# emilk/field_interpolation

Measured on NVIDIA B200. Metric: 3D SDF solve: lattice cells x CG iterations per second, higher is better.
Workload: dtype f32

## Files before the change

### field_interpolation_b200/csrc/solver.cu

```cuda
#include "solver.hpp"

#include <algorithm>
#include <cmath>
#include <cstdlib>

namespace fi {

namespace {

constexpr int kThreads = 256;

int vec_grid(int64_t n)
{
	const int64_t want = (n + kThreads - 1) / kThreads;
	return static_cast<int>(std::max<int64_t>(1, std::min<int64_t>(want, static_cast<int64_t>(sm_count()) * 8)));
}

template <typename T>
struct Pack;
template <>
struct Pack<float>
{
	using type = float4;
	static constexpr int V = 4;
// ... 17 lines not shown
	}
}

template <typename T, typename F>
__device__ __forceinline__ void for_each_pack_blocked(int64_t n, int64_t* first, int64_t* last, F&& f)
{
	constexpr int V      = Pack<T>::V;
	const int64_t npacks = n / V;
	const int64_t chunk  = (npacks + gridDim.x - 1) / gridDim.x;
	const int64_t k0 = static_cast<int64_t>(blockIdx.x) * chunk, k1 = min(k0 + chunk, npacks);
	for (int64_t k = k0 + threadIdx.x; k < k1; k += blockDim.x) { f(k, true); }
	*first = k0 * V;
	*last  = k1 * V;
	if (blockIdx.x == gridDim.x - 1) {
		for (int64_t i = npacks * V + threadIdx.x; i < n; i += blockDim.x) { f(i, false); }
		*last = n;
	}
}

template <typename T>
__global__ void __launch_bounds__(kThreads) pcg_init_kernel(int64_t n, const T* __restrict__ b, const T* __restrict__ q,
                                                            const T* __restrict__ minv, T* __restrict__ r, T* __restrict__ p,
                                                            PcgState* st, double tol, long long max_iters, double* partial,
                                                            unsigned* ticket, int dist)
{
	__shared__ double red[32];
	double            acc[3] = {0, 0, 0};
	const int64_t     stride = static_cast<int64_t>(gridDim.x) * blockDim.x;
	for (int64_t i = static_cast<int64_t>(blockIdx.x) * blockDim.x + threadIdx.x; i < n; i += stride) {
		const T bi = b[i], ri = q ? bi - q[i] : bi, zi = minv[i] * ri;
		r[i] = ri;
		p[i] = zi;
		acc[0] += static_cast<double>(ri) * static_cast<double>(zi);
		acc[1] += static_cast<double>(ri) * static_cast<double>(ri);
		acc[2] += static_cast<double>(bi) * static_cast<double>(bi);
	}
	acc[0] = block_sum(acc[0], red);
	acc[1] = block_sum(acc[1], red);
	acc[2] = block_sum(acc[2], red);
	grid_sum<3>(acc, partial, ticket, red, [&](const double(&tot)[3]) {
		if (dist) {
			st->part[0] = tot[0];
			st->part[1] = tot[1];
			st->part[2] = tot[2];
			return;
		}
		st->rho[0]    = tot[0];
		st->rho[1]    = 0;
		st->pq        = 0;
		st->rr        = tot[1];
		st->rr0       = tot[1];
		st->bb        = tot[2];
		st->tol2bb    = tol * tol * tot[2];
		st->iters     = 0;
// ... 138 lines not shown
	});
	acc[0] = block_sum(acc[0], red);
	acc[1] = block_sum(acc[1], red);
	grid_sum<2>(acc, partial, ticket, red, [&](const double(&tot)[2]) {
		if (XM == kXSkip) { st->alpha_prev = alpha_d; }
		if (dist) {
			st->part[0] = tot[0];
			st->part[1] = tot[1];
			return;
		}
		st->rho[par ^ 1] = tot[0];
		st->rr           = tot[1];
		st->iters += 1;
		if (tot[1] <= st->tol2bb || st->iters >= st->max_iters || !(tot[0] > 0.0)) { st->done = 1; }
	});
}

template <typename T>
struct DirRing
{
	const T* p[kMaxXRing];
};

template <typename T, int M, bool PACKED>
__device__ __forceinline__ void ring_update_elements(int64_t k, T* __restrict__ x, T* __restrict__ r, const DirRing<T>& d, const T* __restrict__ q,
                                                     const T* __restrict__ minv, T alpha, const T (&a)[kMaxXRing], double (&acc)[2])
{
	using P         = typename Pack<T>::type;
	constexpr int V = PACKED ? Pack<T>::V : 1;
	constexpr int MD = M > 0 ? M : 1;
	T ra[V], qa[V], ma[V], xa[V], da[MD][V];
	if (PACKED) {
		*reinterpret_cast<P*>(ra) = reinterpret_cast<const P*>(r)[k];
		*reinterpret_cast<P*>(qa) = reinterpret_cast<const P*>(q)[k];
		*reinterpret_cast<P*>(ma) = reinterpret_cast<const P*>(minv)[k];
		if (M > 0) {
			*reinterpret_cast<P*>(xa) = reinterpret_cast<const P*>(x)[k];
#pragma unroll
			for (int j = 0; j < M; ++j) { *reinterpret_cast<P*>(da[j]) = reinterpret_cast<const P*>(d.p[j])[k]; }
		}
	} else {
		ra[0] = r[k];
		qa[0] = q[k];
		ma[0] = minv[k];
		if (M > 0) {
			xa[0] = x[k];
#pragma unroll
			for (int j = 0; j < M; ++j) { da[j][0] = d.p[j][k]; }
		}
	}
#pragma unroll
	for (int e = 0; e < V; ++e) {
		if (M > 0) {
			T s = a[0] * da[0][e];
#pragma unroll
			for (int j = 1; j < M; ++j) { s += a[j] * da[j][e]; }
			xa[e] += s;
		}
		ra[e] -= alpha * qa[e];
		const double rd = static_cast<double>(ra[e]);
		acc[0] += rd * static_cast<double>(ma[e] * ra[e]);
		acc[1] += rd * rd;
	}
	if (PACKED) {
		if (M > 0) { reinterpret_cast<P*>(x)[k] = *reinterpret_cast<const P*>(xa); }
		reinterpret_cast<P*>(r)[k] = *reinterpret_cast<const P*>(ra);
	} else {
		if (M > 0) { x[k] = xa[0]; }
		r[k] = ra[0];
	}
}

template <typename T, int M>
__global__ void __launch_bounds__(kThreads) pcg_update_ring_kernel(int64_t n, T* __restrict__ x, T* __restrict__ r, DirRing<T> d,
                                                                   const T* __restrict__ q, const T* __restrict__ minv, PcgState* st, int par,
                                                                   double* __restrict__ alpha, int pos, double* partial, unsigned* ticket)
{
	__shared__ double red[32];
	if (st->done) { return; }
	const double pq = st->pq;
	if (!(pq > 0.0)) {
		if (blockIdx.x == 0 && threadIdx.x == 0) {
			st->breakdown = 1;
			st->done      = 1;
		}
		return;
	}
	const double alpha_d = st->rho[par] / pq;
	T            a[kMaxXRing];
#pragma unroll
	for (int j = 0; j < kMaxXRing; ++j) { a[j] = j < M - 1 ? static_cast<T>(alpha[j]) : T(0); }
	if (M > 0) { a[M > 0 ? M - 1 : 0] = static_cast<T>(alpha_d); }
	double acc[2] = {0, 0};
	for_each_pack<T>(n, [&](int64_t k, bool packed) {
		if (packed) {
			ring_update_elements<T, M, true>(k, x, r, d, q, minv, static_cast<T>(alpha_d), a, acc);
		} else {
			ring_update_elements<T, M, false>(k, x, r, d, q, minv, static_cast<T>(alpha_d), a, acc);
		}
	});
	acc[0] = block_sum(acc[0], red);
	acc[1] = block_sum(acc[1], red);
	grid_sum<2>(acc, partial, ticket, red, [&](const double(&tot)[2]) {
		if (M == 0) { alpha[pos] = alpha_d; }
		st->rho[par ^ 1] = tot[0];
		st->rr           = tot[1];
		st->iters += 1;
		if (tot[1] <= st->tol2bb || st->iters >= st->max_iters || !(tot[0] > 0.0)) { st->done = 1; }
	});
}

template <typename T, int XM>
__global__ void __launch_bounds__(kThreads) pcg_update_peer_kernel(int64_t n, T* __restrict__ x, T* __restrict__ r,
                                                                   const T* __restrict__ p, const T* __restrict__ p_prev, const T* __restrict__ q,
                                                                   const T* __restrict__ minv, PcgState* st, int par, double* partial,
                                                                   unsigned* ticket, PeerLink L, HaloPush<T> push, unsigned long long base, int fold,
                                                                   int blocked)
{
	__shared__ double red[32];
	__shared__ double s_pq, s_tot[2];
	__shared__ int    s_ok, s_pub;
// ... 185 lines not shown
		FI_REQUIRE(m == 2 || m == 4 || m == 8, FI_ERR_INVALID, "FI_B200_X_RING must be 2, 4 or 8");
	} else {
		int dev = 0, l2 = 0;
		FI_CUDA(cudaGetDevice(&dev));
		FI_CUDA(cudaDeviceGetAttribute(&l2, cudaDevAttrL2CacheSize, dev));
		const size_t l2_bytes = l2 > 0 ? static_cast<size_t>(l2) : static_cast<size_t>(126) << 20;
		if (6 * vec <= l2_bytes) { return 2; }
	}
	size_t free_b = 0, total_b = 0;
	FI_CUDA(cudaMemGetInfo(&free_b, &total_b));
	while (m > 2 && static_cast<size_t>(std::max(0, m - op.work.dirs)) * vec > free_b / 2) { m /= 2; }
	return m;
}

template <typename T>
void ensure_ring(PcgWork<T>& w, size_t n, int m, cudaStream_t s)
{
	for (; w.dirs < m; ++w.dirs) {
		w.dir[w.dirs].resize(n);
		w.dir[w.dirs].zero(s);
	}
}

template <typename T>
void launch_ring_update(PcgWork<T>& w, int m, int pos, int grid, int64_t n, T* x, const T* minv, int par, cudaStream_t s)
{
	DirRing<T> d = {};
	if (pos < m - 1) {
		auto ku = pcg_update_ring_kernel<T, 0>;
		FI_LAUNCH(ku, grid, kThreads, 0, s, n, x, w.r.data(), d, w.q.data(), minv, w.state.data(), par, w.alpha.data(), pos, w.partial.data(),
		          w.ticket.data());
		return;
	}
	for (int j = 0; j < m; ++j) { d.p[j] = w.dir[(j + 1) % m].data(); }
	auto ku = m == 8 ? pcg_update_ring_kernel<T, 8> : m == 4 ? pcg_update_ring_kernel<T, 4> : pcg_update_ring_kernel<T, 2>;
	FI_LAUNCH(ku, grid, kThreads, 0, s, n, x, w.r.data(), d, w.q.data(), minv, w.state.data(), par, w.alpha.data(), pos, w.partial.data(),
	          w.ticket.data());
}

template <typename T>
void ensure_work(Operator<T>& op, cudaStream_t s)
{
	PcgWork<T>& w = op.work;
	const size_t n = static_cast<size_t>(op.g.N);
	if (w.r.size() != n) {
		w.r.resize(n);
		w.q.resize(n);
		for (int j = 2; j < kMaxXRing; ++j) { w.dir[j].release(); }
		w.dirs = 0;
		ensure_ring(w, n, 2, s);
		w.alpha.resize(kMaxXRing - 1);
		if (op.g.sharded()) {
			w.r.zero(s);
			w.q.zero(s);
		}
		w.partial.resize(static_cast<size_t>(3) * (static_cast<size_t>(sm_count()) * 8 + 8));
		w.ticket.resize(1);
		w.state.resize(1);
		w.ticket.zero(s);
	}
// ... 72 lines not shown
PcgResult pcg_solve(Operator<T>& op, const T* b, T* x, double tol, long long max_iter, int check_every, bool want_true_residual,
                    cudaStream_t s)
{
	TraceScope trace("pcg_solve");
	ensure_work(op, s);
	PcgWork<T>&   w = op.work;
	const int64_t off = op.g.own_offset(), n = op.g.own_cells();
	DistHooks*    dist = op.dist;
	const T*      rhs = b ? b : op.atb.data();
	if (max_iter <= 0) {
		max_iter = 2 * static_cast<long long>(op.g.size[0]) * op.g.size[1] * op.g.size[2];
	}
	if (!(tol > 0)) { tol = std::is_same<T, float>::value ? 1.1920929e-07 : 2.220446049250313e-16; }
	const int ring = choose_x_ring(op);
	ensure_ring(w, static_cast<size_t>(op.g.N), ring, s);
	check_every = std::max(ring, check_every <= 0 ? 32 : check_every);
	check_every = (check_every + ring - 1) / ring * ring;

	cudaEvent_t e0, e1;
	FI_CUDA(cudaEventCreate(&e0));
	FI_CUDA(cudaEventCreate(&e1));
	FI_CUDA(cudaEventRecord(e0, s));

	const int grid = vec_grid(n);
	const PeerLink* link = dist ? dist->link() : nullptr;
	T*              r_vec = w.r.data();
	HaloPush<T>     push;
	if (link) {
		void *lo = nullptr, *hi = nullptr;
		r_vec = static_cast<T*>(dist->shared_vector(static_cast<size_t>(op.g.N) * sizeof(T), &lo, &hi, s));
		const int64_t plane = op.g.stride[2], halo = op.g.zown0;
		push.count = halo * plane;
		if (lo) { push.lo = static_cast<T*>(lo) + halo * plane + dist->peer_own_cells(link->rank - 1); }
		if (hi) { push.hi = static_cast<T*>(hi); }
	}
	const bool zero_guess = op.guess_is_zero;
	op.guess_is_zero      = false;
	if (!zero_guess) {
		if (dist) { dist->exchange_halo(x, sizeof(T), s); }
		op.apply(x, w.q.data(), nullptr, nullptr, s);
	}
	{
		auto kern = pcg_init_kernel<T>;
		FI_LAUNCH(kern, grid, kThreads, 0, s, n, rhs + off, zero_guess ? static_cast<const T*>(nullptr) : w.q.data() + off, op.minv.data() + off, r_vec + off, w.dir[0].data() + off,
		          w.state.data(), tol, max_iter, w.partial.data(), w.ticket.data(), dist ? 1 : 0);
		if (dist) {
			dist->allreduce(w.state.data()->part, 3, s);
			FI_LAUNCH(pcg_init_finish_kernel, 1, 1, 0, s, w.state.data(), tol, max_iter);
			dist->exchange_halo(r_vec, sizeof(T), s);
		}
	}
	PcgState h;
	FI_CUDA(cudaMemcpyAsync(&h, w.state.data(), sizeof(h), cudaMemcpyDeviceToHost, s));
	FI_CUDA(cudaStreamSynchronize(s));

	PcgResult res;
	res.zero_rhs         = (h.bb == 0.0);
	res.initial_residual = h.bb > 0 ? std::sqrt(h.rr0 / h.bb) : 0.0;
	if (res.zero_rhs) {
		FI_CUDA(cudaMemsetAsync(x + off, 0, n * sizeof(T), s));
	} else if (!h.done) {
		const int* d_done = &w.state.data()->done;
		double*    d_pq   = &w.state.data()->pq;
		const unsigned long long seq_base = link ? (dist->next_seq() << 40) : 0ull;
		const char* fold_env  = std::getenv("FI_B200_PEER_FOLD");
		const int   fold_mode = !link ? 0 : (fold_env && *fold_env >= '0' && *fold_env <= '3' ? *fold_env - '0' : 2);
		const bool  data_publishes = fold_mode >= 2, update_finishes = fold_mode == 1 || fold_mode == 2;
		const char* walk_env = std::getenv("FI_B200_PEER_UPDATE");
		const bool  peer_update_blocked = walk_env ? walk_env[0] == 'b' : n < (48ll << 20);
		bool deferred_x = false;
		auto enqueue_round = [&] {
			for (int it = 0; it < check_every; ++it) {
				const int par = it & 1, pos = it % ring;
				T* const   p_old = w.dir[pos].data();
				T* const   p_new = w.dir[(pos + 1) % ring].data();
				const bool fused = stencil_fused_step<T>(op.use_fast, op.g, op.tabs, r_vec, op.minv.data(), p_old, p_new, w.q.data(),
				                                         w.state.data(), par, d_pq, op.partial.data(), op.ticket.data(), d_done, s);
				deferred_x = deferred_x || fused;
				if (fused && link) {
					PeerPublish pub;
					pub.link  = *link;
					pub.which = 0;
					pub.par   = par;
					pub.base  = seq_base;
					pub.st    = w.state.data();
					const bool published = apply_data_term<T>(op.g, op.data, p_new, w.q.data(), d_pq, d_done, s, data_publishes ? &pub : nullptr);
					const bool in_update = fold_mode == 1;
					if (!published && !in_update) { FI_LAUNCH(peer_publish_kernel, 1, 32, 0, s, *link, 0, par, seq_base, w.state.data(), d_pq, 1, d_done); }
					auto ku = par == 0 ? pcg_update_peer_kernel<T, kXSkip> : pcg_update_peer_kernel<T, kXBoth>;
					FI_LAUNCH(ku, grid, kThreads, 0, s, n, x + off, r_vec + off, p_new + off, p_old + off, w.q.data() + off, op.minv.data() + off,
					          w.state.data(), par, w.partial.data(), w.ticket.data(), *link, push, seq_base, (in_update ? 1 : 0) | (update_finishes ? 2 : 0),
					          peer_update_blocked ? 1 : 0);
					if (!update_finishes) { FI_LAUNCH(pcg_update_finish_peer_kernel, 1, 32, 0, s, w.state.data(), par, *link, seq_base); }
				} else if (fused && !dist) {
					apply_data_term<T>(op.g, op.data, p_new, w.q.data(), d_pq, d_done, s);
					launch_ring_update<T>(w, ring, pos, grid, n, x, op.minv.data(), par, s);
				} else if (fused) {
					apply_data_term<T>(op.g, op.data, p_new, w.q.data(), d_pq, d_done, s);
					if (dist) { dist->allreduce(d_pq, 1, s); }
					auto ku = par == 0 ? pcg_update_kernel<T, kXSkip> : pcg_update_kernel<T, kXBoth>;
					FI_LAUNCH(ku, grid, kThreads, 0, s, n, x + off, r_vec + off, p_new + off, p_old + off, w.q.data() + off, op.minv.data() + off,
					          w.state.data(), par, w.partial.data(), w.ticket.data(), dist ? 1 : 0);
					if (dist) {
						dist->allreduce(w.state.data()->part, 2, s);
						FI_LAUNCH(pcg_update_finish_kernel, 1, 1, 0, s, w.state.data(), par);
						dist->exchange_halo(r_vec, sizeof(T), s);
					}
				} else {
					FI_REQUIRE(dist == nullptr, FI_ERR_UNSUPPORTED, "a slab-sharded solve needs the fused 3D stencil kernel");
					T* const p = w.dir[0].data();
					op.apply(p, w.q.data(), d_pq, d_done, s);
					auto ku = pcg_update_kernel<T, kXClassic>;
					FI_LAUNCH(ku, grid, kThreads, 0, s, n, x, w.r.data(), p, static_cast<const T*>(nullptr), w.q.data(), op.minv.data(), w.state.data(), par,
					          w.partial.data(), w.ticket.data(), 0);
					auto kd = pcg_direction_kernel<T>;
					FI_LAUNCH(kd, grid, kThreads, 0, s, n, w.r.data(), op.minv.data(), p, w.state.data(), par);
				}
			}
		};
// ... 194 lines not shown
	h.alpha_prev = 0;
	if (!(h.rho[0] > 0)) { h.rho[0] = 1; }
	if (!(h.rho[1] > 0)) { h.rho[1] = 1; }
	if (!(h.pq > 0)) { h.pq = 1; }
	FI_CUDA(cudaMemcpyAsync(w.state.data(), &h, sizeof(h), cudaMemcpyHostToDevice, s));
	FI_CUDA(cudaStreamSynchronize(s));
	cudaEvent_t e0, e1;
	FI_CUDA(cudaEventCreate(&e0));
	FI_CUDA(cudaEventCreate(&e1));
	auto timed = [&](auto&& body) {
		FI_CUDA(cudaEventRecord(e0, s));
		for (int i = 0; i < iterations; ++i) { body(i); }
		FI_CUDA(cudaEventRecord(e1, s));
		FI_CUDA(cudaEventSynchronize(e1));
		float ms = 0;
		FI_CUDA(cudaEventElapsedTime(&ms, e0, e1));
		return static_cast<double>(ms);
	};
	DevBuf<double> dot(1);
	const int m     = std::max(2, r.x_ring);
	T*        p0    = w.dir[0].data();
	auto      p_old = [&](int i) { return w.dir[i % m].data(); };
	auto      p_new = [&](int i) { return w.dir[(i + 1) % m].data(); };
	bool      fused = false;
	out[1] = timed([&](int i) {
		const int par = i & 1;
		fused = stencil_fused_step<T>(op.use_fast, op.g, op.tabs, w.r.data(), op.minv.data(), p_old(i), p_new(i), w.q.data(),
		                              w.state.data(), par, dot.data(), op.partial.data(), op.ticket.data(), nullptr, s);
		if (fused) {
			apply_data_term<T>(op.g, op.data, p_new(i), w.q.data(), dot.data(), nullptr, s);
		} else {
			op.apply(p0, w.q.data(), dot.data(), nullptr, s);
		}
	});
	h.pq = 1e30;
	FI_CUDA(cudaMemcpyAsync(w.state.data(), &h, sizeof(h), cudaMemcpyHostToDevice, s));
	FI_CUDA(cudaStreamSynchronize(s));
	out[2] = timed([&](int i) {
		if (!fused) {
			auto ku = pcg_update_kernel<T, kXClassic>;
			FI_LAUNCH(ku, vec_grid(n), kThreads, 0, s, n, x.data(), w.r.data(), p0, static_cast<const T*>(nullptr), w.q.data(), op.minv.data(), w.state.data(), 0,
			          w.partial.data(), w.ticket.data(), 0);
		} else {
			launch_ring_update<T>(w, m, i % m, vec_grid(n), n, x.data(), op.minv.data(), 0, s);
		}
	});
	out[3] = 0.0;
	if (!fused) {
		out[3] = timed([&](int) {
			auto kd = pcg_direction_kernel<T>;
			FI_LAUNCH(kd, vec_grid(n), kThreads, 0, s, n, w.r.data(), op.minv.data(), p0, w.state.data(), 0);
		});
	}
	out[4] = fused ? 1.0 : 0.0;
	out[7] = fused ? m : 1;
	out[5] = timed([&](int i) {
		const int par = i & 1;
		if (fused) {
			stencil_fused_step<T>(op.use_fast, op.g, op.tabs, w.r.data(), op.minv.data(), p_old(i), p_new(i), w.q.data(), w.state.data(), par,
			                      dot.data(), op.partial.data(), op.ticket.data(), nullptr, s);
		} else {
			stencil_apply<T>(op.g, op.tabs, p0, w.q.data(), dot.data(), op.partial.data(), op.ticket.data(), nullptr, op.use_fast, s);
		}
	});
	out[6] = timed([&](int i) {
		apply_data_term<T>(op.g, op.data, fused ? p_new(i) : p0, w.q.data(), dot.data(), nullptr, s);
	});
	cudaEventDestroy(e0);
	cudaEventDestroy(e1);
}

template void time_kernels<float>(Operator<float>&, int, int, double*, cudaStream_t);
template void time_kernels<double>(Operator<double>&, int, int, double*, cudaStream_t);
template std::unique_ptr<Operator<float>> build_operator<float>(const Geom&, const ModelAccum&, const PointStore&, const HostRows&, cudaStream_t);
template std::unique_ptr<Operator<double>> build_operator<double>(const Geom&, const ModelAccum&, const PointStore&, const HostRows&, cudaStream_t);
template PcgResult pcg_solve<float>(Operator<float>&, const float*, float*, double, long long, int, bool, cudaStream_t);
template PcgResult pcg_solve<double>(Operator<double>&, const double*, double*, double, long long, int, bool, cudaStream_t);
template PcgResult tile_phase<float>(Operator<float>&, int, float*, double, long long, int, cudaStream_t);
template PcgResult tile_phase<double>(Operator<double>&, int, double*, double, long long, int, cudaStream_t);
template void jacobi_sweeps<float>(Operator<float>&, float*, int, float, cudaStream_t);
template void jacobi_sweeps<double>(Operator<double>&, double*, int, double, cudaStream_t);
template void residual<float>(Operator<float>&, const float*, const float*, float*, double*, double*, cudaStream_t);
// ... 4 lines not shown
```

### field_interpolation_b200/csrc/solver.hpp

```cpp
#pragma once

#include <utility>
#include <vector>

#include "internal.hpp"
#include "peer.cuh"

namespace fi {

struct DistHooks
{
	virtual ~DistHooks() = default;
	virtual const PeerLink* link() { return nullptr; }
	virtual void* shared_vector(size_t bytes, void** lo, void** hi, cudaStream_t s)
	{
		(void)bytes; (void)lo; (void)hi; (void)s;
		return nullptr;
	}
	virtual int64_t peer_own_cells(int peer) { (void)peer; return 0; }
	virtual unsigned long long next_seq() { return 0; }
	virtual void allreduce(double* d_ptr, int count, cudaStream_t s) = 0;
	virtual void exchange_halo(void* d_vec, size_t elem_size, cudaStream_t s) = 0;
	virtual int rank() const { return 0; }
	virtual int world() const { return 1; }
// ... 50 lines not shown

struct PcgResult
{
	long long iterations = 0;
	double    rel_residual = 0, initial_residual = 0, true_residual = 0, solve_ms = 0;
	double    loop_ms = 0;
	int       x_ring = 1;
	bool      converged = false, zero_rhs = false;
	bool      stalled = false;
};

constexpr double kConvergedSlack = 1.25;

template <typename T>
PcgResult pcg_solve(Operator<T>& op, const T* b, T* x, double tol, long long max_iter, int check_every, bool want_true_residual,
                    cudaStream_t s);

template <typename T>
bool stencil_fast_3d_fused(const Geom& g, const StencilTables& t, const T* r, const T* minv, const T* p_old, T* p_new, T* q,
                           const PcgState* st, int par, double* d_dot_out, double* d_partial, unsigned* d_ticket, const int* d_done,
                           cudaStream_t s);

template <typename T>
bool stencil_tma_3d_fused(const Geom& g, const StencilTables& t, const T* r, const T* minv, const T* p_old, T* p_new, T* q,
                          const PcgState* st, int par, double* d_dot_out, double* d_partial, unsigned* d_ticket, const int* d_done,
                          cudaStream_t s);

template <typename T>
bool stencil_tma_3d_epilogue(const Geom& g, const StencilTables& t, const T* in, const T* res_in, T* res_out, const T* minv, T* e, T* d_new,
                             T a, T b, cudaStream_t s);

template <typename T>
bool stencil_tma_2d_fused(const Geom& g, const StencilTables& t, const T* r, const T* minv, const T* p_old, T* p_new, T* q, const PcgState* st, int par,
                          double* d_dot_out, double* d_partial, unsigned* d_ticket, const int* d_done, cudaStream_t s);
template <typename T>
bool stencil_tma_2d_epilogue(const Geom& g, const StencilTables& t, const T* in, const T* res_in, T* res_out, const T* minv, T* e, T* d_new, T a, T b,
                             cudaStream_t s);

template <typename T>
inline bool stencil_fused_step(int mode, const Geom& g, const StencilTables& t, const T* r, const T* minv, const T* p_old, T* p_new,
                               T* q, const PcgState* st, int par, double* d_dot_out, double* d_partial, unsigned* d_ticket,
                               const int* d_done, cudaStream_t s)
{
	if (g.tile) { return false; }
	if (mode == kStencilAuto && g.ndim == 2) { return stencil_tma_2d_fused<T>(g, t, r, minv, p_old, p_new, q, st, par, d_dot_out, d_partial, d_ticket, d_done, s); }
	if (mode == kStencilAuto && stencil_tma_3d_fused<T>(g, t, r, minv, p_old, p_new, q, st, par, d_dot_out, d_partial, d_ticket, d_done, s)) { return true; }
	if (mode != kStencilGeneric && stencil_fast_3d_fused<T>(g, t, r, minv, p_old, p_new, q, st, par, d_dot_out, d_partial, d_ticket, d_done, s)) { return true; }
	return false;
}

struct MgOptions
{
	int    nu               = 3;
	int    nu_coarse        = 0;
	int    gamma            = 1;
	int    w_levels         = 3;
	double cheb_ratio       = 12.0;
	int    coarsest_cells   = 600;
	int    power_iterations = 20;
	int    tail_cells       = 0;
};

inline MgOptions default_mg_options(const ModelAccum& m, const Geom& g, bool sharded, int user_nu, double user_ratio)
{
	MgOptions o;
	const bool high_order = m.on[3] || m.on[4];
	o.nu        = high_order ? 5 : 2;
	o.nu_coarse = high_order ? 0 : 4;
	const int64_t cells = static_cast<int64_t>(g.size[0]) * g.size[1] * g.size[2];
// ... 99 lines not shown
```

### field_interpolation_b200/csrc/stencil_tma.cu

```cuda
#include <cstdlib>
#include <type_traits>

#include "solver.hpp"
#include "tma.cuh"

namespace fi {

namespace {

using namespace tma;

template <typename T, int R, int TY_ = 8>
struct Tile
{
	static constexpr int V    = 16 / sizeof(T);
	static constexpr int NP   = (R + V - 1) / V;
	static constexpr int TXP  = 32;
	static constexpr int TY   = TY_;
	static constexpr int BXP  = TXP + 2 * NP;
	static constexpr int BY   = TY + 2 * R;
	__host__ __device__ static constexpr int ring(bool gs) { return R + 2 + (gs ? 1 : 0); }
	static constexpr int TILE_BYTES = ((BXP * BY * 16 + 127) / 128) * 128;
	static constexpr int BOX_BYTES  = BXP * BY * 16;
};

template <typename T, int R, int S, bool Fused, bool GS, int TY = 8>
constexpr size_t smem_bytes()
{
	using G = Tile<T, R, TY>;
	return 128  + static_cast<size_t>(S) * (Fused ? 3 : 1) * G::TILE_BYTES + static_cast<size_t>(G::ring(GS)) * G::TILE_BYTES +
	       S * sizeof(uint64_t) + 9 * (2 * R + 1) * sizeof(T) + 32 * sizeof(double) + 64;
}

template <typename T, int R, int S, bool Fused, int MINB, bool Epi, bool GS, int TY>
__global__ void __launch_bounds__(256, MINB)
    stencil3d_tma_kernel(const __grid_constant__ CUtensorMap map_a,
                         const __grid_constant__ CUtensorMap map_b,
                         const __grid_constant__ CUtensorMap map_c,
                         int nx, int ny, int nzl, int zo0, int zo1, int zoff, int nzg, int zchunk, TmaTables<T> tab, T gs2,
                         T* __restrict__ q, T* __restrict__ p_new,
                         const PcgState* st, int par, double* dot_out, double* partial, unsigned* ticket, const int* done, EpiArgs<T> epi)
{
	static_assert(!(Fused && Epi), "the epilogue mode takes a plain input");
	using G           = Tile<T, R, TY>;
	constexpr int V   = G::V;
	constexpr int NP  = G::NP;
	constexpr int NA  = Fused ? 3 : 1;
	constexpr int W   = 2 * R + 1;
	constexpr int RING = G::ring(GS);
	using Pack        = typename PackOf<T>::type;
	using PU          = PackU<T, V>;

	if (done && *done) { return; }

#ifdef FI_B200_EMU
	unsigned char* smem_raw = ::cuda_emu::dynamic_smem();
#else
	extern __shared__ unsigned char smem_raw[];
#endif
	unsigned char* base = smem_raw + ((128u - (smem_u32(smem_raw) & 127u)) & 127u);
	auto stage_ptr = [&](int s, int a) { return reinterpret_cast<Pack*>(base + (static_cast<size_t>(s) * NA + a) * G::TILE_BYTES); };
	unsigned char* ring_base = base + static_cast<size_t>(S) * NA * G::TILE_BYTES;
	auto ring_ptr = [&](int slot) { return reinterpret_cast<Pack*>(ring_base + static_cast<size_t>(slot) * G::TILE_BYTES); };
	uint64_t* full  = reinterpret_cast<uint64_t*>(ring_base + static_cast<size_t>(RING) * G::TILE_BYTES);
	T*        zband = reinterpret_cast<T*>(full + S);
	double*   red   = reinterpret_cast<double*>((reinterpret_cast<uintptr_t>(zband + 9 * W) + 7) & ~uintptr_t(7));

	const int tid = threadIdx.x, tx = tid & 31, ty = tid >> 5;
	const int x0t = blockIdx.x * (G::TXP * V);
	const int y0t = blockIdx.y * G::TY;
// ... 26 lines not shown
	}
	{
		const int cls = row_class(min(y, ny - 1), ny);
#pragma unroll
		for (int t = 0; t < W; ++t) { cy[t] = tab.band[1][cls][t + 4 - R]; }
	}
	T lx0[V], ly0 = T(0);
	if (GS) {
#pragma unroll
		for (int j = 0; j < V; ++j) {
			const int xi = min(x0 + j, nx - 1);
			lx0[j]       = static_cast<T>((xi > 0 ? 1 : 0) + (xi < nx - 1 ? 1 : 0));
		}
		const int yi = min(y, ny - 1);
		ly0          = static_cast<T>((yi > 0 ? 1 : 0) + (yi < ny - 1 ? 1 : 0));
	}

	const int lp0    = zb - R;
	const int n_iter = ze + R - lp0;
	auto issue = [&](int i) {
		const int s = i % S;
		mbar_expect_tx(&full[s], NA * G::BOX_BYTES);
		tma_load_3d(stage_ptr(s, 0), &map_a, &full[s], x0t - NP * V, y0t - R, lp0 + i);
		if (Fused) {
			tma_load_3d(stage_ptr(s, 1), &map_b, &full[s], x0t - NP * V, y0t - R, lp0 + i);
			tma_load_3d(stage_ptr(s, 2), &map_c, &full[s], x0t - NP * V, y0t - R, lp0 + i);
		}
	};
	__syncthreads();
	if (tid == 0) {
		for (int i = 0; i < S && i < n_iter; ++i) { issue(i); }
	}

	const bool has_yh = ty < 2 * R;
	const int  yh_row = ty < R ? ty : G::TY + ty;
	const bool has_xh = tid < 2 * NP * G::TY;
	const int  xh_r   = (tid / (2 * NP)) + R;
	const int  xh_k   = tid % (2 * NP);
	const int  xh_col = xh_k < NP ? xh_k : G::TXP + xh_k;
	const int  own_at = (ty + R) * G::BXP + tx + NP;
	const int  yh_at  = yh_row * G::BXP + tx + NP;
	const int  xh_at  = xh_r * G::BXP + xh_col;
	const bool has_ch = GS && has_yh && tx < 2 * NP;
	const int  ch_at  = yh_row * G::BXP + (tx < NP ? tx : G::TXP + tx);

	auto direction = [&](const Pack* sa, const Pack* sb, const Pack* sc, int at) -> Pack {
		if (!Fused) { return sa[at]; }
		PU rr, mm, pp, out;
		rr.v = sa[at];
		mm.v = sb[at];
		pp.v = sc[at];
#pragma unroll
		for (int j = 0; j < V; ++j) { out.a[j] = mm.a[j] * rr.a[j] + beta * pp.a[j]; }
		return out.v;
	};

	PU     pipe[W];
	double acc = 0.0;
	T*       qout = q + static_cast<size_t>(y) * nx + x0;
	T*       pout = Fused ? p_new + static_cast<size_t>(y) * nx + x0 : nullptr;

	PU         pre_r, pre_m, pre_e;
	const bool epi_upd = Epi && epi.d_new != nullptr;
	const size_t xy_off = static_cast<size_t>(y) * nx + x0;
	auto epi_load = [&](int z) {
		const size_t at = static_cast<size_t>(z) * plane + xy_off;
		pre_r.v = *reinterpret_cast<const Pack*>(epi.res_in + at);
		if (epi_upd) {
			pre_m.v = *reinterpret_cast<const Pack*>(epi.minv + at);
			pre_e.v = *reinterpret_cast<const Pack*>(epi.e + at);
		}
	};
	if (Epi && in_xy && zb < ze) { epi_load(zb); }

	int stage = 0, slot = 0;
	uint32_t phase = 0;
	for (int i0 = 0; i0 < n_iter; i0 += W) {
#pragma unroll
		for (int k = 0; k < W; ++k) {
			const int i = i0 + k;
			if (i >= n_iter) { break; }
			const int lp = lp0 + i;
			mbar_wait(&full[stage], phase);
			const Pack* sa = stage_ptr(stage, 0);
			const Pack* sb = Fused ? stage_ptr(stage, 1) : nullptr;
			const Pack* sc = Fused ? stage_ptr(stage, 2) : nullptr;
			Pack*       rg = ring_ptr(slot);
			if (has_own) {
				pipe[k].v  = direction(sa, sb, sc, own_at);
				rg[own_at] = pipe[k].v;
			}
			if (has_yh) { rg[yh_at] = direction(sa, sb, sc, yh_at); }
			if (has_xh) { rg[xh_at] = direction(sa, sb, sc, xh_at); }
			if (has_ch) { rg[ch_at] = direction(sa, sb, sc, ch_at); }
			if (Fused && in_xy && lp >= wlo && lp < whi) { *reinterpret_cast<Pack*>(pout + static_cast<size_t>(lp) * plane) = pipe[k].v; }
			__syncthreads();
			if (tid == 0 && i + S < n_iter) { issue(i + S); }

			const int z = lp - R;
			if (z >= zb && in_xy) {
				int zslot = slot - R;
				if (zslot < 0) { zslot += RING; }
				const Pack* pz = ring_ptr(zslot);
				const T*    cz = zband + row_class(z + zoff, nzg) * W;
				const PU&   ctr = pipe[(k + 1 + R) % W];
				PU          out;
				PU          cur_r, cur_m, cur_e;
				if (Epi) {
					cur_r = pre_r;
// ... 145 lines not shown
inline double plan_chunks(const Geom& g, int R, int S, int minb, int tx_cells, int ty, int* out_chunks)
{
	const int     tiles_x = div_up(g.size[0], tx_cells), tiles_y = div_up(g.size[1], ty);
	const int64_t resident = static_cast<int64_t>(sm_count()) * minb;
	const int64_t tiles    = static_cast<int64_t>(tiles_x) * tiles_y;
	const int     nown     = g.zown1 - g.zown0;
	int           chunks   = 1;
	double        best     = 1e300;
	for (int c = 1; c <= std::max(1, nown / (2 * R + 1)) && c <= 256; ++c) {
		const int     zc    = div_up(nown, c);
		const int     cc    = div_up(nown, zc);
		const int64_t waves = (tiles * cc + resident - 1) / resident;
		const double  frac  = static_cast<double>(tiles * cc) / static_cast<double>(resident);
		const double  cost  = std::max(static_cast<double>(waves) - 0.5, frac) * (zc + 2 * R + S + 1);
		if (cost < best - 1e-9) {
			best   = cost;
			chunks = cc;
		}
	}
	*out_chunks = chunks;
	return best;
}

template <typename T, int R, int S, bool Fused, int MINB, bool Epi, bool GS, int TY>
void launch_ty(const Geom& g, const StencilTables& t, int chunks, const T* a, const T* b, const T* c, T* q, T* p_new, const PcgState* st, int par,
               double* d_dot_out, double* d_partial, unsigned* d_ticket, const int* d_done, cudaStream_t s, const EpiArgs<T>& epi)
{
	using G = Tile<T, R, TY>;
	TmaTables<T> tab;
	for (int ax = 0; ax < kMaxDim; ++ax) {
		for (int cl = 0; cl < 9; ++cl) {
			for (int k = 0; k < 9; ++k) { tab.band[ax][cl][k] = static_cast<T>(t.band[ax][cl][k]); }
		}
	}
	const CUtensorMap ma = make_map<T, R, TY>(g, a);
	const CUtensorMap mb = Fused ? make_map<T, R, TY>(g, b) : ma;
	const CUtensorMap mc = Fused ? make_map<T, R, TY>(g, c) : ma;
	const int tiles_x = div_up(g.size[0], G::TXP * G::V), tiles_y = div_up(g.size[1], G::TY);
	const int nown    = g.zown1 - g.zown0;
	const int zchunk  = div_up(nown, chunks);
	chunks            = div_up(nown, zchunk);
	dim3 grid(tiles_x, tiles_y, chunks);
	auto kern = stencil3d_tma_kernel<T, R, S, Fused, MINB, Epi, GS, TY>;
	constexpr size_t smem = smem_bytes<T, R, S, Fused, GS, TY>();
	static bool configured = false;
	if (!configured) {
		FI_CUDA(cudaFuncSetAttribute(kern, cudaFuncAttributeMaxDynamicSharedMemorySize, static_cast<int>(smem)));
		configured = true;
	}
	FI_LAUNCH(kern, grid, 256, smem, s, ma, mb, mc, g.size[0], g.size[1], g.nzl, g.zown0, g.zown1, g.zoff, g.size[2], zchunk, tab,
	          static_cast<T>(t.gs2), q, p_new, st, par, d_dot_out, d_partial, d_ticket, d_done, epi);
}

template <typename T, int R, int S, bool Fused, int MINB, bool Epi, bool GS>
void launch_gs(const Geom& g, const StencilTables& t, const T* a, const T* b, const T* c, T* q, T* p_new, const PcgState* st, int par,
               double* d_dot_out, double* d_partial, unsigned* d_ticket, const int* d_done, cudaStream_t s, const EpiArgs<T>& epi = EpiArgs<T>())
{
	using G8 = Tile<T, R, 8>;
	int c8 = 1, c7 = 1;
	plan_chunks(g, R, S, MINB, G8::TXP * G8::V, 8, &c8);
	bool seven = false;
	if (R <= 2) {
		static const int forced = [] {
			const char* e = getenv("FI_B200_STENCIL_TY");
			return e ? atoi(e) : 0;
		}();
		plan_chunks(g, R, S, MINB, G8::TXP * G8::V, 7, &c7);
		auto busiest = [&](int ty, int chunks) {
			const int64_t blocks = static_cast<int64_t>(div_up(g.size[0], G8::TXP * G8::V)) * div_up(g.size[1], ty) * chunks;
			const int64_t waves  = (blocks + static_cast<int64_t>(sm_count()) * MINB - 1) / (static_cast<int64_t>(sm_count()) * MINB);
			return static_cast<double>(waves) * (div_up(g.zown1 - g.zown0, chunks) + 2 * R + S + 1) * ty;
		};
		seven = forced == 7 || (forced != 8 && busiest(7, c7) < 0.97 * busiest(8, c8));
	}
	if constexpr (R <= 2) {
		if (seven) {
			launch_ty<T, R, S, Fused, MINB, Epi, GS, 7>(g, t, c7, a, b, c, q, p_new, st, par, d_dot_out, d_partial, d_ticket, d_done, s, epi);
			return;
		}
	}
	launch_ty<T, R, S, Fused, MINB, Epi, GS, 8>(g, t, c8, a, b, c, q, p_new, st, par, d_dot_out, d_partial, d_ticket, d_done, s, epi);
}

template <typename T, int R, int S, bool Fused, int MINB, bool Epi = false>
void launch(const Geom& g, const StencilTables& t, const T* a, const T* b, const T* c, T* q, T* p_new, const PcgState* st, int par,
            double* d_dot_out, double* d_partial, unsigned* d_ticket, const int* d_done, cudaStream_t s, const EpiArgs<T>& epi = EpiArgs<T>())
{
	if (t.gs2 != 0.0) {
		launch_gs<T, R, S, Fused, MINB, Epi, true>(g, t, a, b, c, q, p_new, st, par, d_dot_out, d_partial, d_ticket, d_done, s, epi);
	} else {
		launch_gs<T, R, S, Fused, MINB, Epi, false>(g, t, a, b, c, q, p_new, st, par, d_dot_out, d_partial, d_ticket, d_done, s, epi);
	}
}

template <typename T>
bool eligible(const Geom& g, const StencilTables& t)
{
	constexpr int V = 16 / sizeof(T);
	return g.ndim == 3 && t.radius >= 1 && g.size[0] % V == 0 && g.size[0] >= 32 && g.size[1] >= 8 && g.zown1 - g.zown0 >= 1 &&
	       (g.sharded() || g.size[2] >= 8) && encode_fn() != nullptr;
}

template <typename T, bool Fused>
void dispatch(const Geom& g, const StencilTables& t, const T* a, const T* b, const T* c, T* q, T* p_new, const PcgState* st, int par,
              double* d_dot_out, double* d_partial, unsigned* d_ticket, const int* d_done, cudaStream_t s)
{
	if (t.radius <= 1) {
		launch<T, 1, 3, Fused, 2>(g, t, a, b, c, q, p_new, st, par, d_dot_out, d_partial, d_ticket, d_done, s);
	} else if (t.radius == 2) {
		static const int variant = [] {
			const char* e = getenv("FI_B200_STENCIL_VARIANT");
			return e ? atoi(e) : 0;
		}();
		if (variant == 3 && std::is_same<T, float>::value) {
			launch<T, 2, 2, Fused, 3>(g, t, a, b, c, q, p_new, st, par, d_dot_out, d_partial, d_ticket, d_done, s);
		} else if (variant == 4 && std::is_same<T, float>::value) {
			launch<T, 2, 4, Fused, 2>(g, t, a, b, c, q, p_new, st, par, d_dot_out, d_partial, d_ticket, d_done, s);
		} else {
			launch<T, 2, 3, Fused, 2>(g, t, a, b, c, q, p_new, st, par, d_dot_out, d_partial, d_ticket, d_done, s);
		}
	} else {
		launch<T, 4, 2, Fused, 1>(g, t, a, b, c, q, p_new, st, par, d_dot_out, d_partial, d_ticket, d_done, s);
	}
}

}

template <typename T>
bool stencil_tma_3d(const Geom& g, const StencilTables& t, const T* p, T* q, double* d_dot_out, double* d_partial, unsigned* d_ticket,
                    const int* d_done, cudaStream_t s)
{
	if (!eligible<T>(g, t)) { return false; }
	dispatch<T, false>(g, t, p, nullptr, nullptr, q, nullptr, nullptr, 0, d_dot_out, d_partial, d_ticket, d_done, s);
	return true;
}

template <typename T>
bool stencil_tma_3d_fused(const Geom& g, const StencilTables& t, const T* r, const T* minv, const T* p_old, T* p_new, T* q,
                          const PcgState* st, int par, double* d_dot_out, double* d_partial, unsigned* d_ticket, const int* d_done,
                          cudaStream_t s)
{
	if (!eligible<T>(g, t)) { return false; }
	dispatch<T, true>(g, t, r, minv, p_old, q, p_new, st, par, d_dot_out, d_partial, d_ticket, d_done, s);
	return true;
}

template <typename T>
bool stencil_tma_3d_epilogue(const Geom& g, const StencilTables& t, const T* in, const T* res_in, T* res_out, const T* minv, T* e, T* d_new,
                             T a, T b, cudaStream_t s)
{
	if (!eligible<T>(g, t)) { return false; }
	EpiArgs<T> epi;
	epi.res_in  = res_in;
	epi.res_out = res_out;
	epi.minv    = minv;
	epi.e       = e;
	epi.d_new   = d_new;
	epi.a       = a;
	epi.b       = b;
	if (t.radius <= 1) {
		launch<T, 1, 3, false, 2, true>(g, t, in, nullptr, nullptr, nullptr, nullptr, nullptr, 0, nullptr, nullptr, nullptr, nullptr, s, epi);
	} else if (t.radius == 2) {
		launch<T, 2, 3, false, 2, true>(g, t, in, nullptr, nullptr, nullptr, nullptr, nullptr, 0, nullptr, nullptr, nullptr, nullptr, s, epi);
	} else {
		launch<T, 4, 2, false, 1, true>(g, t, in, nullptr, nullptr, nullptr, nullptr, nullptr, 0, nullptr, nullptr, nullptr, nullptr, s, epi);
	}
	return true;
}

template bool stencil_tma_3d_epilogue<float>(const Geom&, const StencilTables&, const float*, const float*, float*, const float*, float*, float*, float, float, cudaStream_t);
template bool stencil_tma_3d<float>(const Geom&, const StencilTables&, const float*, float*, double*, double*, unsigned*, const int*, cudaStream_t);
template bool stencil_tma_3d<double>(const Geom&, const StencilTables&, const double*, double*, double*, double*, unsigned*, const int*, cudaStream_t);
template bool stencil_tma_3d_fused<float>(const Geom&, const StencilTables&, const float*, const float*, const float*, float*, float*, const PcgState*, int, double*, double*, unsigned*, const int*, cudaStream_t);
template bool stencil_tma_3d_fused<double>(const Geom&, const StencilTables&, const double*, const double*, const double*, double*, double*, const PcgState*, int, double*, double*, unsigned*, const int*, cudaStream_t);

}
```

Before: 135.7 billion.

## Store preconditioned residual z instead of r to drop minv stream from TMA stencil

The solver now keeps the preconditioned residual z = Minv*r in the residual buffer for single-device, untiled 3D lattices that the TMA stencil handles. The fused stencil kernel then forms the search direction as z + beta*p, so it no longer issues a TMA load of minv per tile and uses one fewer shared-memory stage buffer. The update kernel applies minv to q and recovers r by dividing z by minv for the dot products. In exchange it adds a per-element division, and it assumes minv is nonzero, which can change rounding.

```diff
diff --git a/field_interpolation_b200/csrc/solver.cu b/field_interpolation_b200/csrc/solver.cu
--- a/field_interpolation_b200/csrc/solver.cu
+++ b/field_interpolation_b200/csrc/solver.cu
@@ -63,14 +63,14 @@
 __global__ void __launch_bounds__(kThreads) pcg_init_kernel(int64_t n, const T* __restrict__ b, const T* __restrict__ q,
                                                             const T* __restrict__ minv, T* __restrict__ r, T* __restrict__ p,
                                                             PcgState* st, double tol, long long max_iters, double* partial,
-                                                            unsigned* ticket, int dist)
+                                                            unsigned* ticket, int dist, int store_z)
 {
 	__shared__ double red[32];
 	double            acc[3] = {0, 0, 0};
 	const int64_t     stride = static_cast<int64_t>(gridDim.x) * blockDim.x;
 	for (int64_t i = static_cast<int64_t>(blockIdx.x) * blockDim.x + threadIdx.x; i < n; i += stride) {
 		const T bi = b[i], ri = q ? bi - q[i] : bi, zi = minv[i] * ri;
-		r[i] = ri;
+		r[i] = store_z ? zi : ri;
 		p[i] = zi;
 		acc[0] += static_cast<double>(ri) * static_cast<double>(zi);
 		acc[1] += static_cast<double>(ri) * static_cast<double>(ri);
@@ -255,7 +255,7 @@
 	const T* p[kMaxXRing];
 };
 
-template <typename T, int M, bool PACKED>
+template <typename T, int M, bool PACKED, bool Z>
 __device__ __forceinline__ void ring_update_elements(int64_t k, T* __restrict__ x, T* __restrict__ r, const DirRing<T>& d, const T* __restrict__ q,
                                                      const T* __restrict__ minv, T alpha, const T (&a)[kMaxXRing], double (&acc)[2])
 {
@@ -290,10 +290,17 @@
 			for (int j = 1; j < M; ++j) { s += a[j] * da[j][e]; }
 			xa[e] += s;
 		}
-		ra[e] -= alpha * qa[e];
-		const double rd = static_cast<double>(ra[e]);
-		acc[0] += rd * static_cast<double>(ma[e] * ra[e]);
-		acc[1] += rd * rd;
+		if (Z) {
+			ra[e] -= alpha * (ma[e] * qa[e]);
+			const double rd = static_cast<double>(ra[e] / ma[e]);
+			acc[0] += rd * static_cast<double>(ra[e]);
+			acc[1] += rd * rd;
+		} else {
+			ra[e] -= alpha * qa[e];
+			const double rd = static_cast<double>(ra[e]);
+			acc[0] += rd * static_cast<double>(ma[e] * ra[e]);
+			acc[1] += rd * rd;
+		}
 	}
 	if (PACKED) {
 		if (M > 0) { reinterpret_cast<P*>(x)[k] = *reinterpret_cast<const P*>(xa); }
@@ -304,7 +311,7 @@
 	}
 }
 
-template <typename T, int M>
+template <typename T, int M, bool Z>
 __global__ void __launch_bounds__(kThreads) pcg_update_ring_kernel(int64_t n, T* __restrict__ x, T* __restrict__ r, DirRing<T> d,
                                                                    const T* __restrict__ q, const T* __restrict__ minv, PcgState* st, int par,
                                                                    double* __restrict__ alpha, int pos, double* partial, unsigned* ticket)
@@ -327,9 +334,9 @@
 	double acc[2] = {0, 0};
 	for_each_pack<T>(n, [&](int64_t k, bool packed) {
 		if (packed) {
-			ring_update_elements<T, M, true>(k, x, r, d, q, minv, static_cast<T>(alpha_d), a, acc);
+			ring_update_elements<T, M, true, Z>(k, x, r, d, q, minv, static_cast<T>(alpha_d), a, acc);
 		} else {
-			ring_update_elements<T, M, false>(k, x, r, d, q, minv, static_cast<T>(alpha_d), a, acc);
+			ring_update_elements<T, M, false, Z>(k, x, r, d, q, minv, static_cast<T>(alpha_d), a, acc);
 		}
 	});
 	acc[0] = block_sum(acc[0], red);
@@ -561,20 +568,36 @@
 	}
 }
 
-template <typename T>
-void launch_ring_update(PcgWork<T>& w, int m, int pos, int grid, int64_t n, T* x, const T* minv, int par, cudaStream_t s)
+template <typename T, bool Z>
+void launch_ring_update_form(PcgWork<T>& w, int m, int pos, int grid, int64_t n, T* x, const T* minv, int par, cudaStream_t s)
 {
 	DirRing<T> d = {};
 	if (pos < m - 1) {
-		auto ku = pcg_update_ring_kernel<T, 0>;
+		auto ku = pcg_update_ring_kernel<T, 0, Z>;
 		FI_LAUNCH(ku, grid, kThreads, 0, s, n, x, w.r.data(), d, w.q.data(), minv, w.state.data(), par, w.alpha.data(), pos, w.partial.data(),
 		          w.ticket.data());
 		return;
 	}
 	for (int j = 0; j < m; ++j) { d.p[j] = w.dir[(j + 1) % m].data(); }
-	auto ku = m == 8 ? pcg_update_ring_kernel<T, 8> : m == 4 ? pcg_update_ring_kernel<T, 4> : pcg_update_ring_kernel<T, 2>;
+	auto ku = m == 8 ? pcg_update_ring_kernel<T, 8, Z> : m == 4 ? pcg_update_ring_kernel<T, 4, Z> : pcg_update_ring_kernel<T, 2, Z>;
 	FI_LAUNCH(ku, grid, kThreads, 0, s, n, x, w.r.data(), d, w.q.data(), minv, w.state.data(), par, w.alpha.data(), pos, w.partial.data(),
 	          w.ticket.data());
+}
+
+template <typename T>
+void launch_ring_update(PcgWork<T>& w, int m, int pos, int grid, int64_t n, T* x, const T* minv, int par, bool z, cudaStream_t s)
+{
+	if (z) {
+		launch_ring_update_form<T, true>(w, m, pos, grid, n, x, minv, par, s);
+	} else {
+		launch_ring_update_form<T, false>(w, m, pos, grid, n, x, minv, par, s);
+	}
+}
+
+template <typename T>
+bool keeps_z(const Operator<T>& op)
+{
+	return op.dist == nullptr && !op.g.tile && op.use_fast == kStencilAuto && op.g.ndim == 3 && stencil_tma_3d_takes<T>(op.g, op.tabs);
 }
 
 template <typename T>
@@ -693,7 +716,8 @@
 	FI_CUDA(cudaEventCreate(&e1));
 	FI_CUDA(cudaEventRecord(e0, s));
 
-	const int grid = vec_grid(n);
+	const int  grid   = vec_grid(n);
+	const bool keep_z = keeps_z(op);
 	const PeerLink* link = dist ? dist->link() : nullptr;
 	T*              r_vec = w.r.data();
 	HaloPush<T>     push;
@@ -714,7 +738,7 @@
 	{
 		auto kern = pcg_init_kernel<T>;
 		FI_LAUNCH(kern, grid, kThreads, 0, s, n, rhs + off, zero_guess ? static_cast<const T*>(nullptr) : w.q.data() + off, op.minv.data() + off, r_vec + off, w.dir[0].data() + off,
-		          w.state.data(), tol, max_iter, w.partial.data(), w.ticket.data(), dist ? 1 : 0);
+		          w.state.data(), tol, max_iter, w.partial.data(), w.ticket.data(), dist ? 1 : 0, keep_z ? 1 : 0);
 		if (dist) {
 			dist->allreduce(w.state.data()->part, 3, s);
 			FI_LAUNCH(pcg_init_finish_kernel, 1, 1, 0, s, w.state.data(), tol, max_iter);
@@ -745,8 +769,9 @@
 				const int par = it & 1, pos = it % ring;
 				T* const   p_old = w.dir[pos].data();
 				T* const   p_new = w.dir[(pos + 1) % ring].data();
-				const bool fused = stencil_fused_step<T>(op.use_fast, op.g, op.tabs, r_vec, op.minv.data(), p_old, p_new, w.q.data(),
+				const bool fused = stencil_fused_step<T>(op.use_fast, op.g, op.tabs, r_vec, keep_z ? nullptr : op.minv.data(), p_old, p_new, w.q.data(),
 				                                         w.state.data(), par, d_pq, op.partial.data(), op.ticket.data(), d_done, s);
+				FI_REQUIRE(fused || !keep_z, FI_ERR_UNSUPPORTED, "the TMA stencil kernel did not take a lattice it was chosen for");
 				deferred_x = deferred_x || fused;
 				if (fused && link) {
 					PeerPublish pub;
@@ -765,7 +790,7 @@
 					if (!update_finishes) { FI_LAUNCH(pcg_update_finish_peer_kernel, 1, 32, 0, s, w.state.data(), par, *link, seq_base); }
 				} else if (fused && !dist) {
 					apply_data_term<T>(op.g, op.data, p_new, w.q.data(), d_pq, d_done, s);
-					launch_ring_update<T>(w, ring, pos, grid, n, x, op.minv.data(), par, s);
+					launch_ring_update<T>(w, ring, pos, grid, n, x, op.minv.data(), par, keep_z, s);
 				} else if (fused) {
 					apply_data_term<T>(op.g, op.data, p_new, w.q.data(), d_pq, d_done, s);
 					if (dist) { dist->allreduce(d_pq, 1, s); }
@@ -1006,10 +1031,12 @@
 	T*        p0    = w.dir[0].data();
 	auto      p_old = [&](int i) { return w.dir[i % m].data(); };
 	auto      p_new = [&](int i) { return w.dir[(i + 1) % m].data(); };
-	bool      fused = false;
+	bool       fused  = false;
+	const bool keep_z = keeps_z(op);
+	const T*   minv_f = keep_z ? nullptr : op.minv.data();
 	out[1] = timed([&](int i) {
 		const int par = i & 1;
-		fused = stencil_fused_step<T>(op.use_fast, op.g, op.tabs, w.r.data(), op.minv.data(), p_old(i), p_new(i), w.q.data(),
+		fused = stencil_fused_step<T>(op.use_fast, op.g, op.tabs, w.r.data(), minv_f, p_old(i), p_new(i), w.q.data(),
 		                              w.state.data(), par, dot.data(), op.partial.data(), op.ticket.data(), nullptr, s);
 		if (fused) {
 			apply_data_term<T>(op.g, op.data, p_new(i), w.q.data(), dot.data(), nullptr, s);
@@ -1026,7 +1053,7 @@
 			FI_LAUNCH(ku, vec_grid(n), kThreads, 0, s, n, x.data(), w.r.data(), p0, static_cast<const T*>(nullptr), w.q.data(), op.minv.data(), w.state.data(), 0,
 			          w.partial.data(), w.ticket.data(), 0);
 		} else {
-			launch_ring_update<T>(w, m, i % m, vec_grid(n), n, x.data(), op.minv.data(), 0, s);
+			launch_ring_update<T>(w, m, i % m, vec_grid(n), n, x.data(), op.minv.data(), 0, keep_z, s);
 		}
 	});
 	out[3] = 0.0;
@@ -1041,7 +1068,7 @@
 	out[5] = timed([&](int i) {
 		const int par = i & 1;
 		if (fused) {
-			stencil_fused_step<T>(op.use_fast, op.g, op.tabs, w.r.data(), op.minv.data(), p_old(i), p_new(i), w.q.data(), w.state.data(), par,
+			stencil_fused_step<T>(op.use_fast, op.g, op.tabs, w.r.data(), minv_f, p_old(i), p_new(i), w.q.data(), w.state.data(), par,
 			                      dot.data(), op.partial.data(), op.ticket.data(), nullptr, s);
 		} else {
 			stencil_apply<T>(op.g, op.tabs, p0, w.q.data(), dot.data(), op.partial.data(), op.ticket.data(), nullptr, op.use_fast, s);
diff --git a/field_interpolation_b200/csrc/solver.hpp b/field_interpolation_b200/csrc/solver.hpp
--- a/field_interpolation_b200/csrc/solver.hpp
+++ b/field_interpolation_b200/csrc/solver.hpp
@@ -96,6 +96,8 @@
                            cudaStream_t s);
 
 template <typename T>
+bool stencil_tma_3d_takes(const Geom& g, const StencilTables& t);
+template <typename T>
 bool stencil_tma_3d_fused(const Geom& g, const StencilTables& t, const T* r, const T* minv, const T* p_old, T* p_new, T* q,
                           const PcgState* st, int par, double* d_dot_out, double* d_partial, unsigned* d_ticket, const int* d_done,
                           cudaStream_t s);
@@ -119,6 +121,7 @@
 	if (g.tile) { return false; }
 	if (mode == kStencilAuto && g.ndim == 2) { return stencil_tma_2d_fused<T>(g, t, r, minv, p_old, p_new, q, st, par, d_dot_out, d_partial, d_ticket, d_done, s); }
 	if (mode == kStencilAuto && stencil_tma_3d_fused<T>(g, t, r, minv, p_old, p_new, q, st, par, d_dot_out, d_partial, d_ticket, d_done, s)) { return true; }
+	if (!minv) { return false; }
 	if (mode != kStencilGeneric && stencil_fast_3d_fused<T>(g, t, r, minv, p_old, p_new, q, st, par, d_dot_out, d_partial, d_ticket, d_done, s)) { return true; }
 	return false;
 }
diff --git a/field_interpolation_b200/csrc/stencil_tma.cu b/field_interpolation_b200/csrc/stencil_tma.cu
--- a/field_interpolation_b200/csrc/stencil_tma.cu
+++ b/field_interpolation_b200/csrc/stencil_tma.cu
@@ -24,15 +24,15 @@
 	static constexpr int BOX_BYTES  = BXP * BY * 16;
 };
 
-template <typename T, int R, int S, bool Fused, bool GS, int TY = 8>
+template <typename T, int R, int S, bool Fused, bool GS, int TY = 8, bool Pre = false>
 constexpr size_t smem_bytes()
 {
 	using G = Tile<T, R, TY>;
-	return 128  + static_cast<size_t>(S) * (Fused ? 3 : 1) * G::TILE_BYTES + static_cast<size_t>(G::ring(GS)) * G::TILE_BYTES +
+	return 128  + static_cast<size_t>(S) * (Fused ? (Pre ? 2 : 3) : 1) * G::TILE_BYTES + static_cast<size_t>(G::ring(GS)) * G::TILE_BYTES +
 	       S * sizeof(uint64_t) + 9 * (2 * R + 1) * sizeof(T) + 32 * sizeof(double) + 64;
 }
 
-template <typename T, int R, int S, bool Fused, int MINB, bool Epi, bool GS, int TY>
+template <typename T, int R, int S, bool Fused, int MINB, bool Epi, bool GS, int TY, bool Pre>
 __global__ void __launch_bounds__(256, MINB)
     stencil3d_tma_kernel(const __grid_constant__ CUtensorMap map_a,
                          const __grid_constant__ CUtensorMap map_b,
@@ -45,7 +45,8 @@
 	using G           = Tile<T, R, TY>;
 	constexpr int V   = G::V;
 	constexpr int NP  = G::NP;
-	constexpr int NA  = Fused ? 3 : 1;
+	constexpr int NA  = Fused ? (Pre ? 2 : 3) : 1;
+	constexpr int IC  = Pre ? 1 : 2;
 	constexpr int W   = 2 * R + 1;
 	constexpr int RING = G::ring(GS);
 	using Pack        = typename PackOf<T>::type;
@@ -118,10 +119,8 @@
 		const int s = i % S;
 		mbar_expect_tx(&full[s], NA * G::BOX_BYTES);
 		tma_load_3d(stage_ptr(s, 0), &map_a, &full[s], x0t - NP * V, y0t - R, lp0 + i);
-		if (Fused) {
-			tma_load_3d(stage_ptr(s, 1), &map_b, &full[s], x0t - NP * V, y0t - R, lp0 + i);
-			tma_load_3d(stage_ptr(s, 2), &map_c, &full[s], x0t - NP * V, y0t - R, lp0 + i);
-		}
+		if (Fused && !Pre) { tma_load_3d(stage_ptr(s, 1), &map_b, &full[s], x0t - NP * V, y0t - R, lp0 + i); }
+		if (Fused) { tma_load_3d(stage_ptr(s, IC), &map_c, &full[s], x0t - NP * V, y0t - R, lp0 + i); }
 	};
 	__syncthreads();
 	if (tid == 0) {
@@ -144,8 +143,13 @@
 		if (!Fused) { return sa[at]; }
 		PU rr, mm, pp, out;
 		rr.v = sa[at];
+		pp.v = sc[at];
+		if (Pre) {
+#pragma unroll
+			for (int j = 0; j < V; ++j) { out.a[j] = rr.a[j] + beta * pp.a[j]; }
+			return out.v;
+		}
 		mm.v = sb[at];
-		pp.v = sc[at];
 #pragma unroll
 		for (int j = 0; j < V; ++j) { out.a[j] = mm.a[j] * rr.a[j] + beta * pp.a[j]; }
 		return out.v;
@@ -179,8 +183,8 @@
 			const int lp = lp0 + i;
 			mbar_wait(&full[stage], phase);
 			const Pack* sa = stage_ptr(stage, 0);
-			const Pack* sb = Fused ? stage_ptr(stage, 1) : nullptr;
-			const Pack* sc = Fused ? stage_ptr(stage, 2) : nullptr;
+			const Pack* sb = Fused && !Pre ? stage_ptr(stage, 1) : nullptr;
+			const Pack* sc = Fused ? stage_ptr(stage, IC) : nullptr;
 			Pack*       rg = ring_ptr(slot);
 			if (has_own) {
 				pipe[k].v  = direction(sa, sb, sc, own_at);
@@ -372,7 +376,7 @@
 	return best;
 }
 
-template <typename T, int R, int S, bool Fused, int MINB, bool Epi, bool GS, int TY>
+template <typename T, int R, int S, bool Fused, int MINB, bool Epi, bool GS, int TY, bool Pre>
 void launch_ty(const Geom& g, const StencilTables& t, int chunks, const T* a, const T* b, const T* c, T* q, T* p_new, const PcgState* st, int par,
                double* d_dot_out, double* d_partial, unsigned* d_ticket, const int* d_done, cudaStream_t s, const EpiArgs<T>& epi)
 {
@@ -384,15 +388,15 @@
 		}
 	}
 	const CUtensorMap ma = make_map<T, R, TY>(g, a);
-	const CUtensorMap mb = Fused ? make_map<T, R, TY>(g, b) : ma;
+	const CUtensorMap mb = Fused && !Pre ? make_map<T, R, TY>(g, b) : ma;
 	const CUtensorMap mc = Fused ? make_map<T, R, TY>(g, c) : ma;
 	const int tiles_x = div_up(g.size[0], G::TXP * G::V), tiles_y = div_up(g.size[1], G::TY);
 	const int nown    = g.zown1 - g.zown0;
 	const int zchunk  = div_up(nown, chunks);
 	chunks            = div_up(nown, zchunk);
 	dim3 grid(tiles_x, tiles_y, chunks);
-	auto kern = stencil3d_tma_kernel<T, R, S, Fused, MINB, Epi, GS, TY>;
-	constexpr size_t smem = smem_bytes<T, R, S, Fused, GS, TY>();
+	auto kern = stencil3d_tma_kernel<T, R, S, Fused, MINB, Epi, GS, TY, Pre>;
+	constexpr size_t smem = smem_bytes<T, R, S, Fused, GS, TY, Pre>();
 	static bool configured = false;
 	if (!configured) {
 		FI_CUDA(cudaFuncSetAttribute(kern, cudaFuncAttributeMaxDynamicSharedMemorySize, static_cast<int>(smem)));
@@ -402,7 +406,7 @@
 	          static_cast<T>(t.gs2), q, p_new, st, par, d_dot_out, d_partial, d_ticket, d_done, epi);
 }
 
-template <typename T, int R, int S, bool Fused, int MINB, bool Epi, bool GS>
+template <typename T, int R, int S, bool Fused, int MINB, bool Epi, bool GS, bool Pre>
 void launch_gs(const Geom& g, const StencilTables& t, const T* a, const T* b, const T* c, T* q, T* p_new, const PcgState* st, int par,
                double* d_dot_out, double* d_partial, unsigned* d_ticket, const int* d_done, cudaStream_t s, const EpiArgs<T>& epi = EpiArgs<T>())
 {
@@ -425,21 +429,21 @@
 	}
 	if constexpr (R <= 2) {
 		if (seven) {
-			launch_ty<T, R, S, Fused, MINB, Epi, GS, 7>(g, t, c7, a, b, c, q, p_new, st, par, d_dot_out, d_partial, d_ticket, d_done, s, epi);
+			launch_ty<T, R, S, Fused, MINB, Epi, GS, 7, Pre>(g, t, c7, a, b, c, q, p_new, st, par, d_dot_out, d_partial, d_ticket, d_done, s, epi);
 			return;
 		}
 	}
-	launch_ty<T, R, S, Fused, MINB, Epi, GS, 8>(g, t, c8, a, b, c, q, p_new, st, par, d_dot_out, d_partial, d_ticket, d_done, s, epi);
-}
-
-template <typename T, int R, int S, bool Fused, int MINB, bool Epi = false>
+	launch_ty<T, R, S, Fused, MINB, Epi, GS, 8, Pre>(g, t, c8, a, b, c, q, p_new, st, par, d_dot_out, d_partial, d_ticket, d_done, s, epi);
+}
+
+template <typename T, int R, int S, bool Fused, int MINB, bool Epi = false, bool Pre = false>
 void launch(const Geom& g, const StencilTables& t, const T* a, const T* b, const T* c, T* q, T* p_new, const PcgState* st, int par,
             double* d_dot_out, double* d_partial, unsigned* d_ticket, const int* d_done, cudaStream_t s, const EpiArgs<T>& epi = EpiArgs<T>())
 {
 	if (t.gs2 != 0.0) {
-		launch_gs<T, R, S, Fused, MINB, Epi, true>(g, t, a, b, c, q, p_new, st, par, d_dot_out, d_partial, d_ticket, d_done, s, epi);
+		launch_gs<T, R, S, Fused, MINB, Epi, true, Pre>(g, t, a, b, c, q, p_new, st, par, d_dot_out, d_partial, d_ticket, d_done, s, epi);
 	} else {
-		launch_gs<T, R, S, Fused, MINB, Epi, false>(g, t, a, b, c, q, p_new, st, par, d_dot_out, d_partial, d_ticket, d_done, s, epi);
+		launch_gs<T, R, S, Fused, MINB, Epi, false, Pre>(g, t, a, b, c, q, p_new, st, par, d_dot_out, d_partial, d_ticket, d_done, s, epi);
 	}
 }
 
@@ -451,26 +455,26 @@
 	       (g.sharded() || g.size[2] >= 8) && encode_fn() != nullptr;
 }
 
-template <typename T, bool Fused>
+template <typename T, bool Fused, bool Pre = false>
 void dispatch(const Geom& g, const StencilTables& t, const T* a, const T* b, const T* c, T* q, T* p_new, const PcgState* st, int par,
               double* d_dot_out, double* d_partial, unsigned* d_ticket, const int* d_done, cudaStream_t s)
 {
 	if (t.radius <= 1) {
-		launch<T, 1, 3, Fused, 2>(g, t, a, b, c, q, p_new, st, par, d_dot_out, d_partial, d_ticket, d_done, s);
+		launch<T, 1, 3, Fused, 2, false, Pre>(g, t, a, b, c, q, p_new, st, par, d_dot_out, d_partial, d_ticket, d_done, s);
 	} else if (t.radius == 2) {
 		static const int variant = [] {
 			const char* e = getenv("FI_B200_STENCIL_VARIANT");
 			return e ? atoi(e) : 0;
 		}();
 		if (variant == 3 && std::is_same<T, float>::value) {
-			launch<T, 2, 2, Fused, 3>(g, t, a, b, c, q, p_new, st, par, d_dot_out, d_partial, d_ticket, d_done, s);
+			launch<T, 2, 2, Fused, 3, false, Pre>(g, t, a, b, c, q, p_new, st, par, d_dot_out, d_partial, d_ticket, d_done, s);
 		} else if (variant == 4 && std::is_same<T, float>::value) {
-			launch<T, 2, 4, Fused, 2>(g, t, a, b, c, q, p_new, st, par, d_dot_out, d_partial, d_ticket, d_done, s);
+			launch<T, 2, 4, Fused, 2, false, Pre>(g, t, a, b, c, q, p_new, st, par, d_dot_out, d_partial, d_ticket, d_done, s);
 		} else {
-			launch<T, 2, 3, Fused, 2>(g, t, a, b, c, q, p_new, st, par, d_dot_out, d_partial, d_ticket, d_done, s);
+			launch<T, 2, 3, Fused, 2, false, Pre>(g, t, a, b, c, q, p_new, st, par, d_dot_out, d_partial, d_ticket, d_done, s);
 		}
 	} else {
-		launch<T, 4, 2, Fused, 1>(g, t, a, b, c, q, p_new, st, par, d_dot_out, d_partial, d_ticket, d_done, s);
+		launch<T, 4, 2, Fused, 1, false, Pre>(g, t, a, b, c, q, p_new, st, par, d_dot_out, d_partial, d_ticket, d_done, s);
 	}
 }
 
@@ -483,6 +487,12 @@
 	if (!eligible<T>(g, t)) { return false; }
 	dispatch<T, false>(g, t, p, nullptr, nullptr, q, nullptr, nullptr, 0, d_dot_out, d_partial, d_ticket, d_done, s);
 	return true;
+}
+
+template <typename T>
+bool stencil_tma_3d_takes(const Geom& g, const StencilTables& t)
+{
+	return eligible<T>(g, t);
 }
 
 template <typename T>
@@ -491,7 +501,11 @@
                           cudaStream_t s)
 {
 	if (!eligible<T>(g, t)) { return false; }
-	dispatch<T, true>(g, t, r, minv, p_old, q, p_new, st, par, d_dot_out, d_partial, d_ticket, d_done, s);
+	if (minv) {
+		dispatch<T, true>(g, t, r, minv, p_old, q, p_new, st, par, d_dot_out, d_partial, d_ticket, d_done, s);
+	} else {
+		dispatch<T, true, true>(g, t, r, nullptr, p_old, q, p_new, st, par, d_dot_out, d_partial, d_ticket, d_done, s);
+	}
 	return true;
 }
 
@@ -521,6 +535,8 @@
 template bool stencil_tma_3d_epilogue<float>(const Geom&, const StencilTables&, const float*, const float*, float*, const float*, float*, float*, float, float, cudaStream_t);
 template bool stencil_tma_3d<float>(const Geom&, const StencilTables&, const float*, float*, double*, double*, unsigned*, const int*, cudaStream_t);
 template bool stencil_tma_3d<double>(const Geom&, const StencilTables&, const double*, double*, double*, double*, unsigned*, const int*, cudaStream_t);
+template bool stencil_tma_3d_takes<float>(const Geom&, const StencilTables&);
+template bool stencil_tma_3d_takes<double>(const Geom&, const StencilTables&);
 template bool stencil_tma_3d_fused<float>(const Geom&, const StencilTables&, const float*, const float*, const float*, float*, float*, const PcgState*, int, double*, double*, unsigned*, const int*, cudaStream_t);
 template bool stencil_tma_3d_fused<double>(const Geom&, const StencilTables&, const double*, const double*, const double*, double*, double*, const PcgState*, int, double*, double*, unsigned*, const int*, cudaStream_t);
 
```

After: 135.4 billion, median of 6. No clear change (-0.2%).
